# sjpark0905/DNA-LDPC-codes

Measured on AMD Instinct MI355X. Metric: decoded codewords/sec (n=18432, m=2048, 50 BP iters) at 1/2/4/8 GPUs; % HBM roofline, higher is better.
Workload: dtype f64; 1 GPU; bsc-p0.02-100k-per-gpu-bp50; code=decode_n18432_m2048_final.pchk (8,72)-regular, E=147456, input=int8 channel codes in HBM + table code*ln49 (LR = host exp), batch_per_gpu=100000, global_batch=100000, max_iter=50, algo=bp, parallelism=dp1 (contiguous codeword shards, no collective), resident_per_pass=192, group_tiles=3, nontemporal_d=False, continuous=True, resident_pool=True, syndrome_split=False

## Files before the change

dna-ldpc-codes_amd/csrc/engine.hip:

```cpp
#include <hip/hip_ext.h>
#include <hip/hip_runtime.h>

#include <algorithm>
#include <cmath>
#include <cstdio>
#include <cstdlib>
#include <cstring>
#include <thread>
#include <type_traits>
#include <utility>

#include "engine.hpp"
#include "kernels.hpp"
#include "kernels_int.hpp"
#include "encode_kernels.hpp"

namespace ldpc {

static_assert(kTile == dev::TILE && kMsaRecPlanes == dev::MSA_REC_PLANES && kMsaErShift == dev::MSA_ER_SHIFT,
              "engine_plan.hpp restates the kernels' layout constants");
constexpr int kProbes = 4;

static thread_local std::string g_err;
void set_error(const std::string& msg) { g_err = msg; }
// ... 282 lines not shown
    size_t fr = 0, tot = 0;
    if (chunk <= 0) LDPC_HIP(hipMemGetInfo(&fr, &tot));
    p = plan_engine(*g, algo, chunk, sched, fr);
    if (p.error) { set_error(p.error); return LDPC_ERR_ARG; }

    if ((rc = dg.build(*g, p.msa_c))) return rc;
    if (p.cont && (rc = lp.build(p, g->N))) return rc;
    const size_t E = (size_t)std::max<int64_t>(g->E, 1), cap = (size_t)p.cap, tiles = (size_t)p.cap_tiles, N = (size_t)g->N;
    if ((rc = dev_alloc(v2c, cap * E))) return rc;
    if (!p.res && (rc = dev_alloc(c2v_buf, p.c2v_bytes / sizeof(double)))) return rc;
    if ((rc = dev_alloc(prior, cap * N)) || (p.msa_c && (rc = dev_alloc(d_sgn, cap * N))) ||
        (rc = dev_alloc(hard, tiles * N)) || (rc = dev_alloc(active, tiles)) || (rc = dev_alloc(iters, cap)) ||
        (rc = dev_alloc(valid, cap)))
        return rc;
    if (algo < LDPC_ALGO_QMSA && (p.res || p.group_tiles < p.cap_tiles)) return probe(kProbes);
    return LDPC_OK;
}

int32_t Engine::flags() const
{
    return (p.nt_d ? LDPC_SCHED_NONTEMPORAL : 0) | (p.cont ? LDPC_SCHED_CONTINUOUS : 0) |
           (p.msa_c ? LDPC_SCHED_MSA_COMPRESSED : 0) | (p.res ? LDPC_SCHED_RESIDENT : 0) |
           (p.syn_blocks > 0 ? LDPC_SCHED_SPLIT_SYNDROME : 0) | (p.first_fp ? LDPC_SCHED_FIRST_FROM_PRIOR : 0) |
           (p.handover ? LDPC_SCHED_HANDOVER : 0) |
           (sched.flags & (LDPC_SCHED_LR_TABLE | LDPC_SCHED_DEBUG_NO_DRAIN | LDPC_SCHED_DEBUG_BAD_LANE));
}

int Engine::probe(int probes)
{
    dev_ptr<double>& pool = p.res ? v2c : c2v_buf;
    std::vector<dev_ptr<double>> cand;
    cand.push_back(std::move(pool));
    size_t best = 0;
    const int rc = time_candidates(probes, cand, &best);
    pool = std::move(cand[best]);
    return rc;
}

int Engine::time_candidates(int probes, std::vector<dev_ptr<double>>& cand, size_t* best)
{
    const size_t E = (size_t)std::max<int64_t>(g->E, 1);
    const size_t bytes = p.res ? (size_t)p.cap * E * sizeof(double) : p.c2v_bytes;
    const unsigned gt = (unsigned)(p.res ? p.cap_tiles : std::min<int64_t>(p.group_tiles, p.cap_tiles));
    hipStream_t s = stream.get();
    LDPC_HIP(hipMemsetAsync((p.res ? cand[0] : v2c).get(), 0, (size_t)gt * 64 * E * sizeof(double), s));
    LDPC_HIP(hipMemsetAsync(prior.get(), 0, (size_t)gt * 64 * g->N * sizeof(double), s));
    LDPC_HIP(hipMemsetAsync(active.get(), 0xff, (size_t)gt * sizeof(uint64_t), s));
// ... 34 lines not shown
}

int Engine::launch_check(double* scratch, int64_t t0, unsigned gt, const dev::ResStep* rstep, bool timing)
{
    using namespace dev;
    const int32_t M = g->M;
    const int64_t E = g->E;
    const bool reg72 = g->regular_dc && g->dc_max == 72;
    const dim3 grid((M + 3) / 4, gt), blk(256);
    const bool msa = algo == LDPC_ALGO_MSA;
    const int kc = timing ? K_UNCOUNTED : K_CHECK;
    int rc = LDPC_OK;
    if (rstep && !reg72) {
        const int cb = gen_bucket(g->dc_max, CheckBuckets{});
        if (!p.res || scratch != v2c.get() || t0 != 0 || !cb) { set_error("resident check: bad state"); return LDPC_ERR_ARG; }
        dispatch(cb, CheckBuckets{}, [&](auto D, auto MSA) {
            rc = launch(kc, (k_check_gr_res<MSA(), D()>), grid, blk, v2c, dg.row_ptr, M, E, *rstep);
        }, msa);
        return rc;
    }
    if (rstep) {
        if (!p.res || p.msa_c || scratch != v2c.get()) { set_error("resident check: bad state"); return LDPC_ERR_ARG; }
        if (msa) return launch(kc, (k_check_msa<72, false, true>), grid, blk, v2c, v2c, active, M, E, t0, *rstep);
        return launch(kc, (k_check_bp<72, false, true>), grid, blk, v2c, v2c, active, M, E, t0, *rstep);
    }
    if (p.msa_c) {
        const dim3 g1((unsigned)((M + 3) / 4) * gt);
        with_bools([&](auto NT) {
            rc = launch(kc, (k_check_msa_c<72, NT()>), g1, blk, v2c, msa_rec(scratch), msa_meta(scratch, p.c2v_tiles, M),
                        active, dg.row_pos, M, E, t0, gt);
        }, p.nt_d);
        return rc;
    }
    if (reg72) {
        with_bools([&](auto NT) {
            if (msa) rc = launch(kc, (k_check_msa<72, NT(), false>), grid, blk, v2c, scratch, active, M, E, t0, ResStep{});
            else rc = launch(kc, (k_check_bp<72, NT(), false>), grid, blk, v2c, scratch, active, M, E, t0, ResStep{});
        }, p.nt_d);
        return rc;
    }
    const bool bp = algo == LDPC_ALGO_BP;
    const bool in_regs = dispatch(gen_bucket(g->dc_max, CheckBuckets{}), CheckBuckets{}, [&](auto D, auto MSA) {
        rc = launch(kc, k_check_gr<MSA(), D()>, grid, blk, v2c, scratch, active, dg.row_ptr, M, E, t0);
    }, !bp);
    if (!in_regs && bp) rc = launch(kc, k_check_bp_gen, grid, blk, v2c, scratch, active, dg.row_ptr, M, E, t0);
    else if (!in_regs) rc = launch(kc, k_check_msa_gen, grid, blk, v2c, scratch, active, dg.row_ptr, M, E, t0);
// ... 9 lines not shown
int Engine::launch_var(double* scratch, int64_t t0, unsigned gt, double* pt, const dev::Refill& rf, bool timing)
{
    using namespace dev;
    const int32_t N = g->N, M = g->M;
    const int64_t E = g->E;
    const bool reg8 = g->regular_dv && g->dv_max == 8;
    const bool cnt = rf.fresh != nullptr;
    const bool pc = cnt && rf.in_code != nullptr;
    const bool inplace = scratch == v2c.get();
    const int kc = timing ? K_UNCOUNTED : K_VAR;
    int rc = LDPC_OK;
    bool ok = true;
    if (p.msa_c) {
        int cpw = std::min(var_cpw_for(rf), 4);
        if (N % (4 * cpw) != 0) cpw = 1;
        const unsigned nb = gt * (unsigned)(N / (4 * cpw));
        const double* rec = msa_rec(scratch);
        const uint16_t* meta = msa_meta(scratch, p.c2v_tiles, M);
        ok = dispatch(cpw, std::integer_sequence<int, 1, 2, 3, 4>{}, [&](auto CPW, auto CONT, auto NT, auto PC) {
            if constexpr (CONT() || !PC())
                rc = launch(kc, (k_var_msa_c<72, 8, CONT(), CPW(), NT(), PC()>), dim3(nb), dim3(256), rec, meta, v2c, prior,
                            hard, d_sgn, active, dg.col_er, pt, N, M, E, t0, (uint32_t)gt, dg.msa_pa, dg.msa_pb, rf);
        }, cnt, p.nt_d, pc);
    } else if (reg8) {
        const int want = var_cpw_for(rf);
        const int cpw = (want != 3 && N % (4 * want) == 0) ? want : 1;
        const dim3 grid((unsigned)((N + 4 * cpw - 1) / (4 * cpw)), gt);
        ok = dispatch(cpw, std::integer_sequence<int, 1, 2, 4, 8>{},
                      [&](auto CPW, auto MSA, auto NT, auto CONT, auto IP, auto PC) {
            if constexpr (!(IP() && NT()) && (CONT() || !PC()))
                rc = launch(kc, (k_var_m<MSA(), 8, NT(), CONT(), CPW(), IP(), PC()>), grid, dim3(256), scratch, v2c, prior,
                            hard, active, dg.col_edge, pt, N, E, t0, rf);
        }, algo == LDPC_ALGO_MSA, p.nt_d && !inplace, cnt, inplace, pc);
    } else {
        const dim3 grid((N + 3) / 4, gt), blk(256);
        const int vb = gen_bucket(g->dv_max, VarBuckets{});
        const bool bp = algo == LDPC_ALGO_BP;
        if (cnt) {
            if (!vb) { set_error("continuous mode needs column degrees <= 32"); return LDPC_ERR_ARG; }
            dispatch(vb, VarBuckets{}, [&](auto D, auto MSA, auto PC, auto IP) {
                rc = launch(kc, (k_var_gr_cont<MSA(), D(), PC(), IP()>), grid, blk, scratch, v2c, prior, hard, active,
                            dg.col_ptr, dg.col_edge, pt, N, E, t0, rf);
            }, algo == LDPC_ALGO_MSA, pc, inplace);
        } else {
            const bool in_regs = dispatch(vb, VarBuckets{}, [&](auto D, auto MSA) {
                rc = launch(kc, k_var_gr<MSA(), D()>, grid, blk, scratch, v2c, prior, hard, active, dg.col_ptr,
// ... 419 lines not shown
```

dna-ldpc-codes_amd/csrc/engine_plan.hpp:

```cpp
#pragma once
#include <algorithm>
#include <cmath>
#include <cstddef>
#include <cstdint>
#include <utility>

#include "../../include/ldpc_amd.h"
#include "graph.hpp"

namespace ldpc {

constexpr int32_t kDefaultGroupTiles = 3;
constexpr int32_t kDefaultMsaGroupTiles = 8;
constexpr int32_t kDefaultVarCpw = 4;
constexpr int32_t kDefaultVarCpwCoded = 2;
constexpr int32_t kDefaultPoolTiles = 3;
constexpr int32_t kDefaultResPoll = 8;
constexpr int32_t kDefaultSynBlocks = 32;
constexpr int64_t kMsaPool = 1024;
constexpr int64_t kResAutoMaxTiles = 4;

constexpr int32_t kDefaultFlags = LDPC_SCHED_NONTEMPORAL | LDPC_SCHED_CONTINUOUS | LDPC_SCHED_MSA_COMPRESSED |
                                  LDPC_SCHED_RESIDENT | LDPC_SCHED_FIRST_FROM_PRIOR | LDPC_SCHED_LR_TABLE |
                                  LDPC_SCHED_HANDOVER;
constexpr int32_t kAllFlags = kDefaultFlags | LDPC_SCHED_DEBUG_NO_DRAIN | LDPC_SCHED_DEBUG_BAD_LANE;

constexpr int32_t kResolved = 1 << 30, kResChosen = 1 << 29;

inline ldpc_schedule resolve_schedule(const ldpc_schedule* s)
{
    ldpc_schedule r{};
    if (s) r = *s;
    r.flags_set &= kAllFlags;
    r.flags = (kDefaultFlags & ~r.flags_set) | (r.flags & r.flags_set);
    r.flags &= kAllFlags;
    r.flags_set = kAllFlags | kResolved | ((r.flags_set & LDPC_SCHED_RESIDENT) ? kResChosen : 0);
    if (r.group_tiles == 0) r.group_tiles = -2;
    if (r.var_cpw < 1 || r.var_cpw > 8 || (r.var_cpw > 4 && r.var_cpw != 8)) r.var_cpw = -2;
    if (r.pool_tiles <= 0) r.pool_tiles = 0;
    if (r.poll_every <= 0) r.poll_every = kDefaultResPoll;
    if (r.syn_blocks <= 0) r.syn_blocks = kDefaultSynBlocks;
    r.syn_blocks = std::min(r.syn_blocks, 256);
    r.reserved = 0;
    return r;
}
inline bool sched_flag(const ldpc_schedule& s, int bit) { return (s.flags & bit) != 0; }

template <int... Ds>
using Buckets = std::integer_sequence<int, Ds...>;
using CheckBuckets = Buckets<8, 16, 32, 48, 64, 96>;
using VarBuckets = Buckets<4, 8, 12, 16, 24, 32>;

template <int... Ds>
inline int gen_bucket(int32_t dmax, Buckets<Ds...>)
{
    int b = 0;
    (void)((dmax <= Ds && (b = Ds, true)) || ...);
    return b;
}

constexpr double kGenPoolBytes = 226e6;
inline int32_t gen_pool_tiles(const HostGraph& g)
{
    const double per_tile = 64.0 * 8.0 * ((double)g.E + (double)g.N);
    return (int32_t)std::max(1.0, std::min(256.0, std::floor(kGenPoolBytes / std::max(per_tile, 1.0))));
}

inline int64_t engine_bytes_per_codeword(const HostGraph& g)
{
    return 2 * g.E * 8 + (int64_t)g.N * 8 + (g.N + 7) / 8 + 8;
}

constexpr int kTile = 64, kMsaRecPlanes = 4, kMsaErShift = 18;

inline size_t msa_scratch_bytes(int64_t tiles, int32_t M)
{
    return (size_t)tiles * M * kTile * (kMsaRecPlanes * sizeof(double) + sizeof(uint16_t));
}

struct EnginePlan {
    bool msa_c = false;
    bool cont = false;
    bool res = false;
    bool handover = false;
    bool nt_d = false;
    bool first_fp = false;
    bool debug_no_drain = false;
    bool debug_bad_lane = false;
    int var_cpw = 4;
    int res_poll = 8;
    int syn_blocks = 0;
    int64_t cap = 0;
    int64_t cap_tiles = 0;
    int64_t group_tiles = 0;
    int64_t c2v_tiles = 0;
    size_t c2v_bytes = 0;
    const char* error = nullptr;
};

inline EnginePlan plan_engine(const HostGraph& g, int algo, int64_t chunk, const ldpc_schedule& s, size_t free_bytes)
{
    EnginePlan p;
    const bool int_algo = algo >= LDPC_ALGO_QMSA;
    const bool reg_72_8 = g.regular_dc && g.dc_max == 72 && g.regular_dv && g.dv_max == 8;
    p.msa_c = algo == LDPC_ALGO_MSA && reg_72_8 && g.N % 16 == 0 && g.E < ((int64_t)1 << kMsaErShift) &&
              sched_flag(s, LDPC_SCHED_MSA_COMPRESSED);
    p.cont = sched_flag(s, LDPC_SCHED_CONTINUOUS) && !int_algo &&
             (reg_72_8 || (g.regular_dv && g.dv_max == 8) || gen_bucket(g.dv_max, VarBuckets{}) != 0);
    const bool gen_res = !reg_72_8 && gen_bucket(g.dc_max, CheckBuckets{}) != 0 &&
                         gen_bucket(g.dv_max, VarBuckets{}) != 0;
    p.res = sched_flag(s, LDPC_SCHED_RESIDENT) && p.cont && !p.msa_c && ((reg_72_8 && g.N % 32 == 0) || gen_res);
    const bool res_chosen = (s.flags_set & kResChosen) != 0;
    if (p.res && !res_chosen && chunk > kResAutoMaxTiles * 64) p.res = false;
    if (p.res && !res_chosen && reg_72_8 && s.pool_tiles <= 0 &&
        64.0 * 8.0 * kDefaultPoolTiles * ((double)g.E + (double)g.N) > 1.15 * kGenPoolBytes)
        p.res = false;
    p.nt_d = sched_flag(s, LDPC_SCHED_NONTEMPORAL) && !p.res;
    p.handover = sched_flag(s, LDPC_SCHED_HANDOVER) && p.res && reg_72_8 &&
                 (algo == LDPC_ALGO_BP || algo == LDPC_ALGO_MSA);
    p.debug_no_drain = sched_flag(s, LDPC_SCHED_DEBUG_NO_DRAIN);
    p.debug_bad_lane = sched_flag(s, LDPC_SCHED_DEBUG_BAD_LANE);
    p.var_cpw = s.var_cpw;
    p.res_poll = s.poll_every;
    if (chunk <= 0) {
        const int64_t ptiles = s.pool_tiles > 0 ? s.pool_tiles : reg_72_8 ? kDefaultPoolTiles : gen_pool_tiles(g);
        const int64_t want = p.res ? 64 * ptiles : (p.msa_c && p.cont) ? kMsaPool : 16384;
        chunk = std::min<int64_t>(want, (int64_t)(free_bytes / 2) / engine_bytes_per_codeword(g));
    }
    p.cap = std::max<int64_t>(64, (chunk + 63) / 64 * 64);
    p.cap_tiles = p.cap / 64;
    if (p.cap_tiles > 65535) { p.error = "chunk too large (max 4194240 codewords)"; return p; }
    int64_t group = s.group_tiles;
    if (group == -2) group = p.msa_c ? kDefaultMsaGroupTiles : kDefaultGroupTiles;
    p.group_tiles = (p.res || group <= 0 || group > p.cap_tiles) ? p.cap_tiles : group;
    if (p.cont) {
        p.syn_blocks = p.res ? 0 : s.syn_blocks;
        p.first_fp = !p.res && reg_72_8 && algo == LDPC_ALGO_BP && sched_flag(s, LDPC_SCHED_FIRST_FROM_PRIOR);
    }
    if (p.res) {
        p.c2v_tiles = p.cap_tiles;
    } else {
        p.c2v_tiles = std::max<int64_t>(p.group_tiles, p.cont ? (p.cap_tiles + 3) / 4 : 0);
// ... 8 lines not shown
```

dna-ldpc-codes_amd/csrc/kernels.hpp:

```cpp
#pragma once
#include <hip/hip_runtime.h>
#include <cstdint>

#include "kargs.hpp"

namespace ldpc {
namespace dev {

constexpr int TILE = 64;

__device__ __forceinline__ int wave_id() { return __builtin_amdgcn_readfirstlane((int)(threadIdx.x >> 6)); }
__device__ __forceinline__ int lane_id() { return (int)(threadIdx.x & 63); }

__device__ __forceinline__ unsigned xcd_block(unsigned b, unsigned nb)
{
    const unsigned q = nb / 8, r = nb % 8, x = b % 8;
    return (x < r ? x * (q + 1) : r * (q + 1) + (x - r) * q) + b / 8;
}

__device__ __forceinline__ uint64_t shfl_xor_u64(uint64_t v, int m)
{
    uint32_t lo = (uint32_t)v, hi = (uint32_t)(v >> 32);
    lo = (uint32_t)__shfl_xor((int)lo, m);
    hi = (uint32_t)__shfl_xor((int)hi, m);
// ... 325 lines not shown
    double s = 1.0;
#pragma unroll
    for (int g = NSEG - 1; g >= 0; --g) {
        double pk[SEG];
        double q = cp[g];
        asm volatile("" : "+v"(q));
#pragma unroll
        for (int i = 0; i < SEG; ++i) {
            const int k = g * SEG + i;
            if (k < DC) { pk[i] = q; q = q * x[k]; }
        }
#pragma unroll
        for (int i = SEG - 1; i >= 0; --i) {
            const int k = g * SEG + i;
            if (k < DC) {
                const double tt = pk[i] * s;
                dst[(size_t)k * TILE] = (1.0 + tt) / (1.0 - tt);
                s = s * x[k];
            }
        }
    }
}

template <int DC, bool NT, bool RES>
__device__ __forceinline__ void check_bp_block(typename Msg<RES>::in dmsg, typename Msg<RES>::out lr_t,
                                               const uint64_t* __restrict__ active, int32_t M, int64_t E,
                                               int64_t t, uint32_t rb, uint32_t nrb, const ResStep& rs)
{
    const int lane = lane_id();
    const int32_t row = (int32_t)rb * 4 + wave_id();
    const uint64_t act = RES ? rs.cs.occupied[t] : active[t];
    const auto src = dmsg + ((size_t)t * E + (size_t)row * DC) * TILE + lane;
    const auto dst = lr_t + (size_t)row * DC * TILE + lane;
    if constexpr (!RES) {
        if (!(row < M && line_occupied(act, lane))) return;
        double x[DC];
        check_bp_load<DC, NT, false>(x, src);
        check_bp_compute<DC, false>(x, dst);
    } else {
        static_assert(DC <= 2 * TILE, "row parity: two gathers per lane");
        const bool occ_l = (act >> lane) & 1ull;
        const int32_t ln0 = rs.cs.lane_n[t * TILE + lane];
        const int64_t b0 = rs.cs.lane_b[t * TILE + lane];
        const uint64_t pend = pend_lanes(rs, t);
        uint64_t par = 0;
        if (row < M && act != 0) {
            const int32_t* __restrict__ cols = rs.col_idx + (size_t)row * DC;
            const int32_t c0 = cols[lane < DC ? lane : DC - 1];
            const int32_t c1 = cols[TILE + lane < DC ? TILE + lane : DC - 1];
            double x[DC];
            check_bp_load<DC, NT, true>(x, src);
            int32_t d0 = c0, d1 = c1;
            asm volatile("" : "+v"(d0), "+v"(d1));
            const uint64_t* __restrict__ h = rs.hard + (size_t)t * rs.N;
            const uint64_t g0 = h[d0];
            const uint64_t g1 = h[d1];
            check_bp_compute<DC, true>(x, dst);
            uint64_t p = (lane < DC ? g0 : 0ull) ^ (TILE + lane < DC ? g1 : 0ull);
#pragma unroll
            for (int off = 32; off > 0; off >>= 1) p ^= shfl_xor_u64(p, off);
            par = p;
        }
        res_arrive(t, act, par, rs, occ_l ? ln0 : 0, occ_l ? b0 : 0, nrb, pend, pend_parity<DC>(rs, t, row, M, pend));
    }
}

template <int DC, bool PC = false>
__global__ __launch_bounds__(256, 2) void k_check_bp_first(const double* __restrict__ prior,
                                                           const int8_t* __restrict__ pcode,
// ... 54 lines not shown
        const int64_t b = sb[l];
        sc[l][lane] = b >= 0 ? in_code[(size_t)b * N + j0 + lane] : (int8_t)0;
    }
    __syncthreads();
    const bool fr = (frm >> lane) & 1ull;
    for (int c = w; c < TILE; c += 4) {
        const int8_t k = sc[lane][c];
        const size_t o = (size_t)t * N + j0 + c;
        pcode[o * TILE + lane] = k;
        const uint64_t m = __ballot(fr && ptab[k + kCodeBias] < 1.0);
        if (lane == 0) hard[o] = (frm == ~0ull) ? m : ((hard[o] & ~frm) | m);
    }
}

template <int DC, bool NT, bool RES>
__global__ __launch_bounds__(256, 2) void k_check_bp(typename Msg<RES>::in dmsg, typename Msg<RES>::out lr,
                                                     const uint64_t* __restrict__ active, int32_t M, int64_t E,
                                                     int64_t t0, ResStep rs)
{
    check_bp_block<DC, NT, RES>(dmsg, lr + (size_t)blockIdx.y * E * TILE, active, M, E, t0 + blockIdx.y, blockIdx.x,
                                gridDim.x, rs);
}

__global__ __launch_bounds__(256) void k_check_bp_gen(const double* __restrict__ dmsg, double* __restrict__ lr,
                                                      const uint64_t* __restrict__ active,
                                                      const int32_t* __restrict__ row_ptr, int32_t M, int64_t E,
                                                      int64_t t0)
{
    const int lane = lane_id();
    const int32_t row = blockIdx.x * 4 + wave_id();
    const int64_t t = t0 + blockIdx.y;
    if (row >= M) return;
    const uint64_t act = active[t];
    if (!((act >> lane) & 1ull)) return;
    const int32_t a = row_ptr[row], b = row_ptr[row + 1];
    const size_t tb = (size_t)t * E, tl = (size_t)blockIdx.y * E;
    double dl = 1.0;
    for (int32_t e = a; e < b; ++e) {
        lr[(tl + e) * TILE + lane] = dl;
        dl = dl * dmsg[(tb + e) * TILE + lane];
    }
    dl = 1.0;
    for (int32_t e = b - 1; e >= a; --e) {
        const size_t o = (tl + e) * TILE + lane;
        const double tt = lr[o] * dl;
        lr[o] = (1.0 + tt) / (1.0 - tt);
        dl = dl * dmsg[(tb + e) * TILE + lane];
    }
}

template <bool PC>
__device__ __forceinline__ double prior_at(const double* __restrict__ prior, const Refill& rf, size_t i)
{
    if constexpr (PC) return rf.ptab[rf.pcode[i] + kCodeBias];
    else return prior[i];
}

template <bool MSA, int DV, bool NT, bool CONT, int CPW, bool INPLACE, bool PC = false>
__device__ __forceinline__ void var_m_block(typename Msg<INPLACE>::in c2v_t, typename Msg<INPLACE>::out v2c,
                                            double* __restrict__ prior, uint64_t* __restrict__ hard,
                                            const uint64_t* __restrict__ active, const int32_t* __restrict__ col_edge,
                                            double* __restrict__ post, int32_t N, int64_t E, int64_t t, uint32_t cb,
                                            const Refill& rf)
{
    const int lane = lane_id();
    const int32_t j0 = ((int32_t)cb * 4 + wave_id()) * CPW;
    if (j0 >= N) return;
    const uint64_t act = active[t];
    const uint64_t frm = CONT ? rf.fresh[t] : 0ull;
    const uint64_t touched = act | frm;
    const uint64_t fm = (CONT && rf.fin) ? rf.fin[t] : 0ull;
    constexpr bool HO = CONT && INPLACE;
    const uint64_t lastm = (HO && rf.last) ? rf.last[t] : 0ull;
    if (touched == 0 && fm == 0) return;
    const bool live = (act >> lane) & 1ull;
    const bool fr = CONT && ((frm >> lane) & 1ull);
    const bool fl = (fm >> lane) & 1ull;
    const bool ls = HO && ((lastm >> lane) & 1ull);
// ... 22 lines not shown
            else xin[c] = rf.in[rb + j0 + c];
        }
    }
    if (live) {
#pragma unroll
        for (int c = 0; c < CPW; ++c) {
            pv[c] = prior_at<PC>(prior, rf, ((size_t)t * N + j0 + c) * TILE + lane);
#pragma unroll
            for (int s = 0; s < DV; ++s) l[c][s] = c2v_t[(size_t)eid[c][s] * TILE + lane];
        }
    }
    if constexpr (PC) {
        if (fr) {
#pragma unroll
            for (int c = 0; c < CPW; ++c) xin[c] = rf.ptab[kin[c] + kCodeBias];
        }
    }
    if (HO && lastm != 0) {
        const int64_t lb = ls ? rf.pend_b[t * TILE + lane] : 0;
        const bool lok = out_ok(lb, rf);
        uint64_t hwf[CPW];
#pragma unroll
        for (int c = 0; c < CPW; ++c) {
            bool hf = false;
            if (ls) {
                double p = pv[c];
                if (MSA) {
#pragma unroll
                    for (int s = 0; s < DV; ++s) p = p + l[c][s];
                    hf = !(p > 0);
                    if (lok && rf.post_out) rf.post_out[(size_t)lb * N + j0 + c] = p;
                } else {
#pragma unroll
                    for (int s = 0; s < DV; ++s) p = p * l[c][s];
                    if (__builtin_isnan(p)) p = 1.0;
                    hf = (p <= 1.0);
                    if (lok && rf.post_out) rf.post_out[(size_t)lb * N + j0 + c] = rf.post_ratio ? p : log(p);
                }
            }
            hwf[c] = __ballot(hf);
            if (lane == 0) rf.hard_fin[(size_t)t * N + j0 + c] = hwf[c];
        }
        if (ls && lok) store_fin_hard<CPW>(rf, hwf, lb, N, j0, lane);
        if (ls && !lok) lane_fault(rf.fault, kFaultOutput, t * TILE + lane);
    }
    const bool fok = out_ok(fb, rf);
    if (CONT && fl && fok) {
        uint64_t hw[CPW];
#pragma unroll
        for (int c = 0; c < CPW; ++c) hw[c] = hard[(size_t)t * N + j0 + c];
        store_fin_hard<CPW>(rf, hw, fb, N, j0, lane);
    }
#pragma unroll
    for (int c = 0; c < CPW; ++c) {
        const int32_t j = j0 + c;
        const size_t pj = ((size_t)t * N + j) * TILE + lane;
        if (CONT && fl && fok && rf.post_out) {
            const size_t ob = (size_t)fb * N + j;
            const double pv = fn > 0 ? post[pj] : prior_at<PC>(prior, rf, pj);
            if (MSA) rf.post_out[ob] = pv;
            else {
                const double P = __builtin_isnan(pv) ? 1.0 : pv;
                rf.post_out[ob] = rf.post_ratio ? P : log(P);
            }
        }
        bool h = false;
        double dv[DV];
#pragma unroll
        for (int s = 0; s < DV; ++s) dv[s] = 0.0;
        double np = 0.0;
        if (live) np = pv[c];
        if (fr) {
            const double x = xin[c];
            if (MSA) {
                np = x;
#pragma unroll
                for (int s = 0; s < DV; ++s) dv[s] = x;
                h = !(x > 0);
            } else {
                const double LR0 = (!PC && rf.in_is_llr) ? exp(x) : x;
                np = LR0;
                const double d0 = 1.0 - 2.0 / (1.0 + LR0);
#pragma unroll
                for (int s = 0; s < DV; ++s) dv[s] = d0;
                h = (LR0 < 1.0);
            }
        } else if (live && !ls) {
            if (MSA) {
#pragma unroll
                for (int s = 0; s < DV; ++s) {
                    double sum = pv[c];
#pragma unroll
                    for (int r = 0; r < DV; ++r)
                        if (r != s) sum = sum + l[c][r];
                    dv[s] = sum;
                }
                double L = pv[c];
#pragma unroll
                for (int s = 0; s < DV; ++s) L = L + l[c][s];
                h = !(L > 0);
                if (post) post[pj] = L;
            } else {
                double pr[DV];
                double p = pv[c];
#pragma unroll
                for (int s = 0; s < DV; ++s) { pr[s] = p; p = p * l[c][s]; }
                if (__builtin_isnan(p)) p = 1.0;
                h = (p <= 1.0);
                if (post) post[pj] = p;
                double acc = 1.0;
#pragma unroll
                for (int s = DV - 1; s >= 0; --s) {
                    double v = pr[s] * acc;
                    if (__builtin_isnan(v)) v = 1.0;
                    acc = acc * l[c][s];
                    dv[s] = 1.0 - 2.0 / (1.0 + v);
                }
            }
        }
        if (CONT && fr) {
            if constexpr (PC) rf.pcode[pj] = kin[c];
            else prior[pj] = np;
        }
        const bool skip_init = CONT && rf.prior_only && !live;
        if (!skip_init && (line_occupied(touched, lane) || fr || live)) {
#pragma unroll
            for (int s = 0; s < DV; ++s) st<NT>(v2c + (tb + eid[c][s]) * TILE + lane, dv[s]);
        }
        const uint64_t m = __ballot(h);
        if (lane == 0 && touched) {
            const size_t o = (size_t)t * N + j;
            const uint64_t old = (touched == ~0ull) ? 0ull : hard[o];
            hard[o] = (old & ~touched) | (m & touched);
        }
    }
    if (CONT && fl && !fok) lane_fault(rf.fault, kFaultOutput, t * TILE + lane);
    asm volatile("" : "+v"(bad_v));
    if (bad_v) lane_fault(rf.fault, kFaultRefill, t * TILE + lane);
}

template <bool MSA, int DV, bool NT, bool CONT, int CPW, bool INPLACE, bool PC = false>
__global__ __launch_bounds__(256) void k_var_m(typename Msg<INPLACE>::in c2v, typename Msg<INPLACE>::out v2c,
                                               double* __restrict__ prior, uint64_t* __restrict__ hard,
                                               const uint64_t* __restrict__ active,
                                               const int32_t* __restrict__ col_edge, double* __restrict__ post,
                                               int32_t N, int64_t E, int64_t t0, Refill rf)
{
    static_assert(CONT || !PC, "coded priors come with continuous refills");
    var_m_block<MSA, DV, NT, CONT, CPW, INPLACE, PC>(c2v + (size_t)blockIdx.y * E * TILE, v2c, prior, hard, active,
                                                 col_edge, post, N, E, t0 + blockIdx.y,
                                                 xcd_block(blockIdx.x, gridDim.x), rf);
}

__device__ __forceinline__ void merge_hard(uint64_t* __restrict__ hard, int64_t t, int32_t N, int32_t j, uint64_t mask,
                                           bool h, int lane)
{
    const uint64_t m = __ballot(h);
    if (lane == 0 && mask) {
        const size_t o = (size_t)t * N + j;
        const uint64_t old = (mask == ~0ull) ? 0ull : hard[o];
        hard[o] = (old & ~mask) | (m & mask);
    }
}

__global__ __launch_bounds__(256) void k_var_bp_gen(const double* __restrict__ lr, double* __restrict__ dmsg,
                                                    const double* __restrict__ prior, uint64_t* __restrict__ hard,
                                                    const uint64_t* __restrict__ active, const int32_t* __restrict__ col_ptr,
                                                    const int32_t* __restrict__ col_edge, double* __restrict__ post,
                                                    int32_t N, int64_t E, int64_t t0)
{
    const int lane = lane_id();
    const int32_t j = blockIdx.x * 4 + wave_id();
    const int64_t t = t0 + blockIdx.y;
    if (j >= N) return;
// ... 973 lines not shown
```

dna-ldpc-codes_amd/ldpc_amd.py:

```python
from __future__ import annotations

import ctypes as C
import enum
import math
import os
import threading
import time
from typing import Optional, Sequence

import numpy as np

_HERE = os.path.dirname(os.path.abspath(__file__))
LIB_PATH = os.path.join(_HERE, "lib", "libldpc_amd.so")

ABI_VERSION = 3
LDPC_OK, LDPC_ERR_ARG, LDPC_ERR_IO, LDPC_ERR_FORMAT, LDPC_ERR_DEVICE, LDPC_ERR_UNSUPPORTED = 0, -1, -2, -3, -4, -5


class Algo(enum.IntEnum):
    BP = 0
    MSA = 1
    QMSA = 2
    GALLAGER_A = 3
    GALLAGER_B1 = 4
# ... 1 lines not shown


ALGO_BP, ALGO_MSA, ALGO_QMSA = Algo.BP, Algo.MSA, Algo.QMSA
ALGO_GALLAGER_A, ALGO_GALLAGER_B1, ALGO_GALLAGER_B2 = Algo.GALLAGER_A, Algo.GALLAGER_B1, Algo.GALLAGER_B2
POST_LLR, POST_RATIO = 0, 1
IN_LLR, IN_LR = 0, 1
H2D, D2H, D2D = 0, 1, 2

_NAMES = {"bp": ALGO_BP, "msa": ALGO_MSA, "min-sum": ALGO_MSA, "qmsa": ALGO_QMSA,
          "gallager_a": ALGO_GALLAGER_A, "gallager_b1": ALGO_GALLAGER_B1, "gallager_b2": ALGO_GALLAGER_B2}
DECODER_TYPES = {0: ALGO_BP, 1: ALGO_GALLAGER_A, 2: ALGO_GALLAGER_B1, 3: ALGO_GALLAGER_B2,
                 20: ALGO_MSA, 21: ALGO_MSA, 22: ALGO_MSA}
_RESULT_TYPE = {ALGO_BP: 0, ALGO_GALLAGER_A: 1, ALGO_GALLAGER_B1: 2, ALGO_GALLAGER_B2: 3, ALGO_MSA: 20,
                ALGO_QMSA: 21}


class LdpcError(RuntimeError):
    def __init__(self, code: int, msg: str):
        super().__init__(f"ldpc_amd error {code}: {msg}")
        self.code = code


SCHED_FLAGS = {"nontemporal": 1 << 0, "continuous": 1 << 3, "msa_compressed": 1 << 4, "resident": 1 << 5,
               "split_syndrome": 1 << 6, "handover": 1 << 7, "first_from_prior": 1 << 12, "lr_table": 1 << 13,
               "debug_no_drain": 1 << 14, "debug_bad_lane": 1 << 15}
SCHED_FIELDS = ("group_tiles", "var_cpw", "pool_tiles", "poll_every", "syn_blocks")


class Schedule(C.Structure):
    _fields_ = [("flags_set", C.c_int32), ("flags", C.c_int32), ("group_tiles", C.c_int32), ("var_cpw", C.c_int32),
                ("pool_tiles", C.c_int32), ("poll_every", C.c_int32), ("syn_blocks", C.c_int32),
                ("reserved", C.c_int32)]

    @classmethod
    def make(cls, **kw) -> "Schedule":
        s = cls()
        for k, v in kw.items():
            if v is None:
                continue
            if k in SCHED_FLAGS:
                s.flags_set |= SCHED_FLAGS[k]
                if v:
                    s.flags |= SCHED_FLAGS[k]
            elif k in SCHED_FIELDS:
                setattr(s, k, int(v))
            else:
                raise TypeError(f"unknown schedule keyword {k!r} (flags: {sorted(SCHED_FLAGS)}, fields: {SCHED_FIELDS})")
# ... 440 lines not shown

class Engine:

    def __init__(self, g: Graph, device: int = 0, algo="bp", chunk: int = 0, schedule=None, **sched_kw):
        self.g, self.device, self.algo = g, device, _algo(algo)
        kw = dict(_schedule_kw(schedule))
        kw.update({k: v for k, v in sched_kw.items() if v is not None})
        sch = Schedule.make(**kw)
        err = C.c_int(0)
        self._h = lib().ldpc_engine_create_ex(g.handle, device, self.algo, chunk, C.byref(sch), C.byref(err))
        if not self._h:
            raise LdpcError(err.value, (lib().ldpc_last_error() or b"").decode())
        cap, grp, fl = C.c_int64(), C.c_int64(), C.c_int32()
        _check(lib().ldpc_engine_info(self._h, C.byref(cap), C.byref(grp), C.byref(fl)))
        self.cap, self.group_tiles, self.flags = cap.value, grp.value, fl.value
        f = fl.value
        self.nontemporal = bool(f & SCHED_FLAGS["nontemporal"])
        self.continuous = bool(f & SCHED_FLAGS["continuous"])
        self.msa_compressed = bool(f & SCHED_FLAGS["msa_compressed"])
        self.resident = bool(f & SCHED_FLAGS["resident"])
        self.syndrome_split = bool(f & SCHED_FLAGS["split_syndrome"])
        self.first_from_prior = bool(f & SCHED_FLAGS["first_from_prior"])
        self.handover = bool(f & SCHED_FLAGS["handover"])

    def decode(self, d_in, in_kind: int, B: int, max_iter: int, d_hard=None, d_post=None, post_kind=POST_LLR,
               d_iters=None, d_valid=None):
        _check(lib().ldpc_engine_decode(self._h, d_in, in_kind, B, max_iter, d_hard, d_post, post_kind, d_iters,
                                        d_valid))

    def decode_codes(self, d_codes, table: np.ndarray, table_kind: int, B: int, max_iter: int, d_hard=None,
                     d_post=None, post_kind=POST_LLR, d_iters=None, d_valid=None):
        t = np.ascontiguousarray(table, dtype=np.float64)
        if t.shape != (256,):
            raise ValueError("the code table has 256 entries (code + 128)")
        _check(lib().ldpc_engine_decode_codes(self._h, d_codes, _ptr(t), table_kind, B, max_iter, d_hard, d_post,
                                              post_kind, d_iters, d_valid))

    def set_params(self, msa_precision: int = 6, msa_step: float = 0.5, msa_offset: int = 0, tie_seed: int = 0):
        _check(lib().ldpc_engine_set_params(self._h, msa_precision, msa_step, msa_offset, tie_seed))

    def gen_bsc(self, d_out, out_kind: int, b0: int, B: int, d_cw, n_cw: int, seed: int, p: float, llr_mag: float):
        _check(lib().ldpc_engine_gen_bsc(self._h, d_out, out_kind, b0, B, d_cw, n_cw, seed, p, llr_mag))

    def gen_bsc_codes(self, d_out, b0: int, B: int, d_cw, n_cw: int, seed: int, p: float):
        _check(lib().ldpc_engine_gen_bsc_codes(self._h, d_out, b0, B, d_cw, n_cw, seed, p))

# ... 94 lines not shown
```

include/ldpc_amd.h:

```cpp
#ifndef LDPC_AMD_H
#define LDPC_AMD_H

#include <stddef.h>
#include <stdint.h>

#ifdef __cplusplus
extern "C" {
#endif

#define LDPC_AMD_ABI_VERSION 3

enum {
    LDPC_OK = 0,
    LDPC_ERR_ARG = -1,
    LDPC_ERR_IO = -2,
    LDPC_ERR_FORMAT = -3,
    LDPC_ERR_DEVICE = -4,
    LDPC_ERR_UNSUPPORTED = -5
};

enum {
    LDPC_ALGO_BP = 0,
    LDPC_ALGO_MSA = 1,
    LDPC_ALGO_QMSA = 2,
// ... 1 lines not shown
    LDPC_ALGO_GALLAGER_B1 = 4,
    LDPC_ALGO_GALLAGER_B2 = 5
};

enum {
    LDPC_POST_LLR = 0,
    LDPC_POST_RATIO = 1
};

enum {
    LDPC_IN_LLR = 0,
    LDPC_IN_LR = 1
};

typedef struct ldpc_graph ldpc_graph;

enum {
    LDPC_SCHED_NONTEMPORAL = 1 << 0,
    LDPC_SCHED_CONTINUOUS = 1 << 3,
    LDPC_SCHED_MSA_COMPRESSED = 1 << 4,
    LDPC_SCHED_RESIDENT = 1 << 5,
    LDPC_SCHED_SPLIT_SYNDROME = 1 << 6,
    LDPC_SCHED_HANDOVER = 1 << 7,
    LDPC_SCHED_FIRST_FROM_PRIOR = 1 << 12,
    LDPC_SCHED_LR_TABLE = 1 << 13,
    LDPC_SCHED_DEBUG_NO_DRAIN = 1 << 14,
    LDPC_SCHED_DEBUG_BAD_LANE = 1 << 15
};

typedef struct ldpc_schedule {
    int32_t flags_set;
    int32_t flags;
    int32_t group_tiles;
    int32_t var_cpw;
    int32_t pool_tiles;
    int32_t poll_every;
    int32_t syn_blocks;
    int32_t reserved;
} ldpc_schedule;

typedef struct ldpc_opts {
    int32_t n_devices;
    const int32_t *devices;
    int64_t chunk;
    int32_t exp_on_host;
    int32_t post_kind;
// ... 239 lines not shown
```

Measured before the change: 27750 codewords/s.

## Fuse check update of one row block into the BP variable kernel

Detects a block of M/8 check rows whose columns each appear exactly once, so every variable node has one edge there. For that block the variable kernel keeps the new variable-to-check messages in shared memory and computes the check-node BP update in the same pass with prefix and suffix products. The check kernel then only computes parity for those rows, which removes one pass over that eighth of the message array. It adds a new kernel path with 8 waves per block and a dependency on the code structure. It is on by default for resident, regular (72,8) BP when the default var_cpw is used.

```diff
diff --git a/dna-ldpc-codes_amd/csrc/engine.hip b/dna-ldpc-codes_amd/csrc/engine.hip
--- a/dna-ldpc-codes_amd/csrc/engine.hip
+++ b/dna-ldpc-codes_amd/csrc/engine.hip
@@ -328,7 +328,7 @@
     return (p.nt_d ? LDPC_SCHED_NONTEMPORAL : 0) | (p.cont ? LDPC_SCHED_CONTINUOUS : 0) |
            (p.msa_c ? LDPC_SCHED_MSA_COMPRESSED : 0) | (p.res ? LDPC_SCHED_RESIDENT : 0) |
            (p.syn_blocks > 0 ? LDPC_SCHED_SPLIT_SYNDROME : 0) | (p.first_fp ? LDPC_SCHED_FIRST_FROM_PRIOR : 0) |
-           (p.handover ? LDPC_SCHED_HANDOVER : 0) |
+           (p.handover ? LDPC_SCHED_HANDOVER : 0) | (p.fuse_block >= 0 ? LDPC_SCHED_FUSE_ROW_BLOCK : 0) |
            (sched.flags & (LDPC_SCHED_LR_TABLE | LDPC_SCHED_DEBUG_NO_DRAIN | LDPC_SCHED_DEBUG_BAD_LANE));
 }
 
@@ -409,6 +409,12 @@
     if (rstep) {
         if (!p.res || p.msa_c || scratch != v2c.get()) { set_error("resident check: bad state"); return LDPC_ERR_ARG; }
         if (msa) return launch(kc, (k_check_msa<72, false, true>), grid, blk, v2c, v2c, active, M, E, t0, *rstep);
+        if (p.fuse_block >= 0) {
+            if (t0 != 0) { set_error("resident check: bad state"); return LDPC_ERR_ARG; }
+            const int32_t Q = M / 8;
+            return launch(kc, (k_check_bp_skip<72>), grid, blk, v2c, v2c, M, E, p.fuse_block * Q, (p.fuse_block + 1) * Q,
+                          *rstep);
+        }
         return launch(kc, (k_check_bp<72, false, true>), grid, blk, v2c, v2c, active, M, E, t0, *rstep);
     }
     if (p.msa_c) {
@@ -464,6 +470,13 @@
                 rc = launch(kc, (k_var_msa_c<72, 8, CONT(), CPW(), NT(), PC()>), dim3(nb), dim3(256), rec, meta, v2c, prior,
                             hard, d_sgn, active, dg.col_er, pt, N, M, E, t0, (uint32_t)gt, dg.msa_pa, dg.msa_pb, rf);
         }, cnt, p.nt_d, pc);
+    } else if (reg8 && p.fuse_block >= 0 && cnt && inplace) {
+        if (t0 != 0 || timing) { set_error("fused row block: bad state"); return LDPC_ERR_ARG; }
+        const dim3 grid((unsigned)(M / 8), gt);
+        with_bools([&](auto PC) {
+            rc = launch(kc, (k_var_bp_fused<kFuseWaves, kFuseCpw, PC()>), grid, dim3(64 * kFuseWaves), v2c, prior, hard,
+                        active, dg.col_edge, dg.col_idx, pt, N, E, p.fuse_block * (M / 8), rf);
+        }, pc);
     } else if (reg8) {
         const int want = var_cpw_for(rf);
         const int cpw = (want != 3 && N % (4 * want) == 0) ? want : 1;
diff --git a/dna-ldpc-codes_amd/csrc/engine_plan.hpp b/dna-ldpc-codes_amd/csrc/engine_plan.hpp
--- a/dna-ldpc-codes_amd/csrc/engine_plan.hpp
+++ b/dna-ldpc-codes_amd/csrc/engine_plan.hpp
@@ -4,6 +4,7 @@
 #include <cstddef>
 #include <cstdint>
 #include <utility>
+#include <vector>
 
 #include "../../include/ldpc_amd.h"
 #include "graph.hpp"
@@ -25,16 +26,18 @@
                                   LDPC_SCHED_HANDOVER;
 constexpr int32_t kAllFlags = kDefaultFlags | LDPC_SCHED_DEBUG_NO_DRAIN | LDPC_SCHED_DEBUG_BAD_LANE;
 
-constexpr int32_t kResolved = 1 << 30, kResChosen = 1 << 29;
+constexpr int32_t kResolved = 1 << 30, kResChosen = 1 << 29, kNoFuse = 1 << 28;
 
 inline ldpc_schedule resolve_schedule(const ldpc_schedule* s)
 {
     ldpc_schedule r{};
     if (s) r = *s;
+    const bool no_fuse = (r.flags_set & LDPC_SCHED_FUSE_ROW_BLOCK) && !(r.flags & LDPC_SCHED_FUSE_ROW_BLOCK);
     r.flags_set &= kAllFlags;
     r.flags = (kDefaultFlags & ~r.flags_set) | (r.flags & r.flags_set);
     r.flags &= kAllFlags;
-    r.flags_set = kAllFlags | kResolved | ((r.flags_set & LDPC_SCHED_RESIDENT) ? kResChosen : 0);
+    r.flags_set = kAllFlags | kResolved | ((r.flags_set & LDPC_SCHED_RESIDENT) ? kResChosen : 0) |
+                  (no_fuse ? kNoFuse : 0);
     if (r.group_tiles == 0) r.group_tiles = -2;
     if (r.var_cpw < 1 || r.var_cpw > 8 || (r.var_cpw > 4 && r.var_cpw != 8)) r.var_cpw = -2;
     if (r.pool_tiles <= 0) r.pool_tiles = 0;
@@ -78,11 +81,32 @@
     return (size_t)tiles * M * kTile * (kMsaRecPlanes * sizeof(double) + sizeof(uint16_t));
 }
 
+inline int fuse_row_block_of(const HostGraph& g)
+{
+    const int dv = g.dv_max;
+    if (dv <= 0 || g.M % dv != 0 || !g.regular_dc) return -1;
+    const int32_t Q = g.M / dv;
+    if ((int64_t)Q * g.dc_max != g.N) return -1;
+    std::vector<uint8_t> seen((size_t)g.N);
+    for (int a = 0; a < dv; a++) {
+        std::fill(seen.begin(), seen.end(), (uint8_t)0);
+        bool once = true;
+        for (int64_t e = (int64_t)a * Q * g.dc_max; once && e < (int64_t)(a + 1) * Q * g.dc_max; e++) {
+            uint8_t& c = seen[(size_t)g.col_idx[(size_t)e]];
+            once = c == 0;
+            c = 1;
+        }
+        if (once) return a;
+    }
+    return -1;
+}
+
 struct EnginePlan {
     bool msa_c = false;
     bool cont = false;
     bool res = false;
     bool handover = false;
+    int fuse_block = -1;
     bool nt_d = false;
     bool first_fp = false;
     bool debug_no_drain = false;
@@ -118,6 +142,8 @@
     p.nt_d = sched_flag(s, LDPC_SCHED_NONTEMPORAL) && !p.res;
     p.handover = sched_flag(s, LDPC_SCHED_HANDOVER) && p.res && reg_72_8 &&
                  (algo == LDPC_ALGO_BP || algo == LDPC_ALGO_MSA);
+    if (!(s.flags_set & kNoFuse) && p.res && reg_72_8 && algo == LDPC_ALGO_BP && s.var_cpw == -2)
+        p.fuse_block = fuse_row_block_of(g);
     p.debug_no_drain = sched_flag(s, LDPC_SCHED_DEBUG_NO_DRAIN);
     p.debug_bad_lane = sched_flag(s, LDPC_SCHED_DEBUG_BAD_LANE);
     p.var_cpw = s.var_cpw;
diff --git a/dna-ldpc-codes_amd/csrc/kernels.hpp b/dna-ldpc-codes_amd/csrc/kernels.hpp
--- a/dna-ldpc-codes_amd/csrc/kernels.hpp
+++ b/dna-ldpc-codes_amd/csrc/kernels.hpp
@@ -371,11 +371,13 @@
     }
 }
 
-template <int DC, bool NT, bool RES>
+template <int DC, bool NT, bool RES, bool SKIP = false>
 __device__ __forceinline__ void check_bp_block(typename Msg<RES>::in dmsg, typename Msg<RES>::out lr_t,
                                                const uint64_t* __restrict__ active, int32_t M, int64_t E,
-                                               int64_t t, uint32_t rb, uint32_t nrb, const ResStep& rs)
-{
+                                               int64_t t, uint32_t rb, uint32_t nrb, const ResStep& rs,
+                                               int32_t skip_lo = 0, int32_t skip_hi = 0)
+{
+    static_assert(RES || !SKIP, "rows are skipped in the resident pool only");
     const int lane = lane_id();
     const int32_t row = (int32_t)rb * 4 + wave_id();
     const uint64_t act = RES ? rs.cs.occupied[t] : active[t];
@@ -393,7 +395,9 @@
         const int64_t b0 = rs.cs.lane_b[t * TILE + lane];
         const uint64_t pend = pend_lanes(rs, t);
         uint64_t par = 0;
-        if (row < M && act != 0) {
+        if (SKIP && row >= skip_lo && row < skip_hi) {
+            if (act != 0) par = row_parity<DC>(rs.hard + (size_t)t * rs.N, rs.col_idx + (size_t)row * DC);
+        } else if (row < M && act != 0) {
             const int32_t* __restrict__ cols = rs.col_idx + (size_t)row * DC;
             const int32_t c0 = cols[lane < DC ? lane : DC - 1];
             const int32_t c1 = cols[TILE + lane < DC ? TILE + lane : DC - 1];
@@ -494,6 +498,14 @@
                                 gridDim.x, rs);
 }
 
+template <int DC>
+__global__ __launch_bounds__(256, 2) void k_check_bp_skip(const double* dmsg, double* lr, int32_t M, int64_t E,
+                                                          int32_t skip_lo, int32_t skip_hi, ResStep rs)
+{
+    check_bp_block<DC, false, true, true>(dmsg, lr + (size_t)blockIdx.y * E * TILE, nullptr, M, E, blockIdx.y,
+                                          blockIdx.x, gridDim.x, rs, skip_lo, skip_hi);
+}
+
 __global__ __launch_bounds__(256) void k_check_bp_gen(const double* __restrict__ dmsg, double* __restrict__ lr,
                                                       const uint64_t* __restrict__ active,
                                                       const int32_t* __restrict__ row_ptr, int32_t M, int64_t E,
@@ -526,6 +538,111 @@
 {
     if constexpr (PC) return rf.ptab[rf.pcode[i] + kCodeBias];
     else return prior[i];
+}
+
+template <bool MSA, int DV>
+__device__ __forceinline__ bool var_column_final(bool ls, double pvc, const double (&l)[DV], bool lok,
+                                                 const Refill& rf, int64_t lb, int32_t N, int32_t j)
+{
+    bool hf = false;
+    if (ls) {
+        double p = pvc;
+        if (MSA) {
+#pragma unroll
+            for (int s = 0; s < DV; ++s) p = p + l[s];
+            hf = !(p > 0);
+            if (lok && rf.post_out) rf.post_out[(size_t)lb * N + j] = p;
+        } else {
+#pragma unroll
+            for (int s = 0; s < DV; ++s) p = p * l[s];
+            if (__builtin_isnan(p)) p = 1.0;
+            hf = (p <= 1.0);
+            if (lok && rf.post_out) rf.post_out[(size_t)lb * N + j] = rf.post_ratio ? p : log(p);
+        }
+    }
+    return hf;
+}
+
+template <bool MSA, bool PC>
+__device__ __forceinline__ void var_column_fin_post(const Refill& rf, const double* __restrict__ prior,
+                                                    const double* post, size_t pj, size_t ob, int32_t fn)
+{
+    const double pv = fn > 0 ? post[pj] : prior_at<PC>(prior, rf, pj);
+    if (MSA) rf.post_out[ob] = pv;
+    else {
+        const double P = __builtin_isnan(pv) ? 1.0 : pv;
+        rf.post_out[ob] = rf.post_ratio ? P : log(P);
+    }
+}
+
+template <bool MSA, int DV, bool PC>
+__device__ __forceinline__ void var_column(bool live, bool fr, bool ls, double pvc, double x, const double (&l)[DV],
+                                           const Refill& rf, double* post, size_t pj, double (&dv)[DV], double& np,
+                                           bool& h)
+{
+    h = false;
+#pragma unroll
+    for (int s = 0; s < DV; ++s) dv[s] = 0.0;
+    np = 0.0;
+    if (live) np = pvc;
+    if (fr) {
+        if (MSA) {
+            np = x;
+#pragma unroll
+            for (int s = 0; s < DV; ++s) dv[s] = x;
+            h = !(x > 0);
+        } else {
+            const double LR0 = (!PC && rf.in_is_llr) ? exp(x) : x;
+            np = LR0;
+            const double d0 = 1.0 - 2.0 / (1.0 + LR0);
+#pragma unroll
+            for (int s = 0; s < DV; ++s) dv[s] = d0;
+            h = (LR0 < 1.0);
+        }
+    } else if (live && !ls) {
+        if (MSA) {
+#pragma unroll
+            for (int s = 0; s < DV; ++s) {
+                double sum = pvc;
+#pragma unroll
+                for (int r = 0; r < DV; ++r)
+                    if (r != s) sum = sum + l[r];
+                dv[s] = sum;
+            }
+            double L = pvc;
+#pragma unroll
+            for (int s = 0; s < DV; ++s) L = L + l[s];
+            h = !(L > 0);
+            if (post) post[pj] = L;
+        } else {
+            double pr[DV];
+            double p = pvc;
+#pragma unroll
+            for (int s = 0; s < DV; ++s) { pr[s] = p; p = p * l[s]; }
+            if (__builtin_isnan(p)) p = 1.0;
+            h = (p <= 1.0);
+            if (post) post[pj] = p;
+            double acc = 1.0;
+#pragma unroll
+            for (int s = DV - 1; s >= 0; --s) {
+                double v = pr[s] * acc;
+                if (__builtin_isnan(v)) v = 1.0;
+                acc = acc * l[s];
+                dv[s] = 1.0 - 2.0 / (1.0 + v);
+            }
+        }
+    }
+}
+
+__device__ __forceinline__ void merge_touched(uint64_t* __restrict__ hard, int64_t t, int32_t N, int32_t j,
+                                              uint64_t touched, bool h, int lane)
+{
+    const uint64_t m = __ballot(h);
+    if (lane == 0 && touched) {
+        const size_t o = (size_t)t * N + j;
+        const uint64_t old = (touched == ~0ull) ? 0ull : hard[o];
+        hard[o] = (old & ~touched) | (m & touched);
+    }
 }
 
 template <bool MSA, int DV, bool NT, bool CONT, int CPW, bool INPLACE, bool PC = false>
@@ -594,22 +711,7 @@
         uint64_t hwf[CPW];
 #pragma unroll
         for (int c = 0; c < CPW; ++c) {
-            bool hf = false;
-            if (ls) {
-                double p = pv[c];
-                if (MSA) {
-#pragma unroll
-                    for (int s = 0; s < DV; ++s) p = p + l[c][s];
-                    hf = !(p > 0);
-                    if (lok && rf.post_out) rf.post_out[(size_t)lb * N + j0 + c] = p;
-                } else {
-#pragma unroll
-                    for (int s = 0; s < DV; ++s) p = p * l[c][s];
-                    if (__builtin_isnan(p)) p = 1.0;
-                    hf = (p <= 1.0);
-                    if (lok && rf.post_out) rf.post_out[(size_t)lb * N + j0 + c] = rf.post_ratio ? p : log(p);
-                }
-            }
+            const bool hf = var_column_final<MSA, DV>(ls, pv[c], l[c], lok, rf, lb, N, j0 + c);
             hwf[c] = __ballot(hf);
             if (lane == 0) rf.hard_fin[(size_t)t * N + j0 + c] = hwf[c];
         }
@@ -627,69 +729,11 @@
     for (int c = 0; c < CPW; ++c) {
         const int32_t j = j0 + c;
         const size_t pj = ((size_t)t * N + j) * TILE + lane;
-        if (CONT && fl && fok && rf.post_out) {
-            const size_t ob = (size_t)fb * N + j;
-            const double pv = fn > 0 ? post[pj] : prior_at<PC>(prior, rf, pj);
-            if (MSA) rf.post_out[ob] = pv;
-            else {
-                const double P = __builtin_isnan(pv) ? 1.0 : pv;
-                rf.post_out[ob] = rf.post_ratio ? P : log(P);
-            }
-        }
-        bool h = false;
-        double dv[DV];
-#pragma unroll
-        for (int s = 0; s < DV; ++s) dv[s] = 0.0;
-        double np = 0.0;
-        if (live) np = pv[c];
-        if (fr) {
-            const double x = xin[c];
-            if (MSA) {
-                np = x;
-#pragma unroll
-                for (int s = 0; s < DV; ++s) dv[s] = x;
-                h = !(x > 0);
-            } else {
-                const double LR0 = (!PC && rf.in_is_llr) ? exp(x) : x;
-                np = LR0;
-                const double d0 = 1.0 - 2.0 / (1.0 + LR0);
-#pragma unroll
-                for (int s = 0; s < DV; ++s) dv[s] = d0;
-                h = (LR0 < 1.0);
-            }
-        } else if (live && !ls) {
-            if (MSA) {
-#pragma unroll
-                for (int s = 0; s < DV; ++s) {
-                    double sum = pv[c];
-#pragma unroll
-                    for (int r = 0; r < DV; ++r)
-                        if (r != s) sum = sum + l[c][r];
-                    dv[s] = sum;
-                }
-                double L = pv[c];
-#pragma unroll
-                for (int s = 0; s < DV; ++s) L = L + l[c][s];
-                h = !(L > 0);
-                if (post) post[pj] = L;
-            } else {
-                double pr[DV];
-                double p = pv[c];
-#pragma unroll
-                for (int s = 0; s < DV; ++s) { pr[s] = p; p = p * l[c][s]; }
-                if (__builtin_isnan(p)) p = 1.0;
-                h = (p <= 1.0);
-                if (post) post[pj] = p;
-                double acc = 1.0;
-#pragma unroll
-                for (int s = DV - 1; s >= 0; --s) {
-                    double v = pr[s] * acc;
-                    if (__builtin_isnan(v)) v = 1.0;
-                    acc = acc * l[c][s];
-                    dv[s] = 1.0 - 2.0 / (1.0 + v);
-                }
-            }
-        }
+        if (CONT && fl && fok && rf.post_out)
+            var_column_fin_post<MSA, PC>(rf, prior, post, pj, (size_t)fb * N + j, fn);
+        bool h;
+        double dv[DV], np;
+        var_column<MSA, DV, PC>(live, fr, ls, pv[c], xin[c], l[c], rf, post, pj, dv, np, h);
         if (CONT && fr) {
             if constexpr (PC) rf.pcode[pj] = kin[c];
             else prior[pj] = np;
@@ -699,12 +743,7 @@
 #pragma unroll
             for (int s = 0; s < DV; ++s) st<NT>(v2c + (tb + eid[c][s]) * TILE + lane, dv[s]);
         }
-        const uint64_t m = __ballot(h);
-        if (lane == 0 && touched) {
-            const size_t o = (size_t)t * N + j;
-            const uint64_t old = (touched == ~0ull) ? 0ull : hard[o];
-            hard[o] = (old & ~touched) | (m & touched);
-        }
+        merge_touched(hard, t, N, j, touched, h, lane);
     }
     if (CONT && fl && !fok) lane_fault(rf.fault, kFaultOutput, t * TILE + lane);
     asm volatile("" : "+v"(bad_v));
@@ -722,6 +761,154 @@
     var_m_block<MSA, DV, NT, CONT, CPW, INPLACE, PC>(c2v + (size_t)blockIdx.y * E * TILE, v2c, prior, hard, active,
                                                  col_edge, post, N, E, t0 + blockIdx.y,
                                                  xcd_block(blockIdx.x, gridDim.x), rf);
+}
+
+constexpr int kFuseWaves = 8, kFuseCpw = 3;
+template <int W, int CPW, bool PC>
+__global__ __launch_bounds__(64 * W) void k_var_bp_fused(double* msg, double* __restrict__ prior,
+                                                         uint64_t* __restrict__ hard,
+                                                         const uint64_t* __restrict__ active,
+                                                         const int32_t* __restrict__ col_edge,
+                                                         const int32_t* __restrict__ col_idx, double* post, int32_t N,
+                                                         int64_t E, int32_t row0, Refill rf)
+{
+    constexpr int DC = 72, DV = 8, KW = DC / W;
+    static_assert(DC % W == 0 && KW % CPW == 0, "the row's columns split evenly over the waves and their rounds");
+    __shared__ double sd[DC][TILE];
+    const int lane = lane_id(), w = wave_id();
+    const int64_t t = blockIdx.y;
+    const int32_t row = row0 + (int32_t)xcd_block(blockIdx.x, gridDim.x);
+    const uint64_t act = active[t];
+    const uint64_t frm = rf.fresh[t];
+    const uint64_t touched = act | frm;
+    const uint64_t fm = rf.fin ? rf.fin[t] : 0ull;
+    const uint64_t lastm = rf.last ? rf.last[t] : 0ull;
+    if (touched == 0 && fm == 0) return;
+    const bool live = (act >> lane) & 1ull;
+    const bool fr = (frm >> lane) & 1ull;
+    const bool fl = (fm >> lane) & 1ull;
+    const bool ls = (lastm >> lane) & 1ull;
+    int64_t fb = 0;
+    int32_t fn = 0;
+    if (fl) {
+        fb = rf.fin_b[t * TILE + lane];
+        fn = rf.fin_n[t * TILE + lane];
+    }
+    double* m_t = msg + (size_t)t * E * TILE;
+    const int k0 = w * KW;
+    const int32_t e0 = row * DC + k0;
+    bool bad_in = false;
+    int bad_v = 0;
+    size_t rb = 0;
+    if (fr) {
+        rb = (size_t)refill_row(rf.lane_b[t * TILE + lane], rf, bad_in) * N;
+        bad_v = bad_in ? 1 : 0;
+    }
+    const int64_t lb = ls ? rf.pend_b[t * TILE + lane] : 0;
+    const bool lok = out_ok(lb, rf), fok = out_ok(fb, rf);
+    const bool keep = line_occupied(touched, lane) || fr || live;
+#pragma unroll
+    for (int r = 0; r < KW; r += CPW) {
+        int32_t j[CPW], eid[CPW][DV];
+#pragma unroll
+        for (int c = 0; c < CPW; ++c) j[c] = col_idx[e0 + r + c];
+#pragma unroll
+        for (int c = 0; c < CPW; ++c)
+#pragma unroll
+            for (int s = 0; s < DV; ++s) eid[c][s] = col_edge[(size_t)j[c] * DV + s];
+        double l[CPW][DV], pv[CPW], xin[CPW];
+        int8_t kin[CPW];
+        if (fr) {
+#pragma unroll
+            for (int c = 0; c < CPW; ++c) {
+                if constexpr (PC) kin[c] = rf.in_code[rb + j[c]];
+                else xin[c] = rf.in[rb + j[c]];
+            }
+        }
+        if (live) {
+#pragma unroll
+            for (int c = 0; c < CPW; ++c) {
+                pv[c] = prior_at<PC>(prior, rf, ((size_t)t * N + j[c]) * TILE + lane);
+#pragma unroll
+                for (int s = 0; s < DV; ++s) l[c][s] = m_t[(size_t)eid[c][s] * TILE + lane];
+            }
+        }
+        if constexpr (PC) {
+            if (fr) {
+#pragma unroll
+                for (int c = 0; c < CPW; ++c) xin[c] = rf.ptab[kin[c] + kCodeBias];
+            }
+        }
+        if (lastm != 0) {
+#pragma unroll
+            for (int c = 0; c < CPW; ++c) {
+                const uint64_t hwf = __ballot(var_column_final<false, DV>(ls, pv[c], l[c], lok, rf, lb, N, j[c]));
+                if (lane == 0) rf.hard_fin[(size_t)t * N + j[c]] = hwf;
+                if (ls && lok) store_fin_hard<1>(rf, &hwf, lb, N, j[c], lane);
+            }
+        }
+        if (fl && fok) {
+#pragma unroll
+            for (int c = 0; c < CPW; ++c) {
+                const uint64_t hw = hard[(size_t)t * N + j[c]];
+                store_fin_hard<1>(rf, &hw, fb, N, j[c], lane);
+            }
+        }
+#pragma unroll
+        for (int c = 0; c < CPW; ++c) {
+            const size_t pj = ((size_t)t * N + j[c]) * TILE + lane;
+            if (fl && fok && rf.post_out) var_column_fin_post<false, PC>(rf, prior, post, pj, (size_t)fb * N + j[c], fn);
+            bool h;
+            double dv[DV], np;
+            var_column<false, DV, PC>(live, fr, ls, pv[c], xin[c], l[c], rf, post, pj, dv, np, h);
+            if (fr) {
+                if constexpr (PC) rf.pcode[pj] = kin[c];
+                else prior[pj] = np;
+            }
+            const int32_t ea = e0 + r + c;
+            if (keep) {
+#pragma unroll
+                for (int s = 0; s < DV; ++s) {
+                    if (eid[c][s] == ea) sd[k0 + r + c][lane] = dv[s];
+                    else m_t[(size_t)eid[c][s] * TILE + lane] = dv[s];
+                }
+            }
+            merge_touched(hard, t, N, j[c], touched, h, lane);
+        }
+    }
+    if (lastm != 0 && ls && !lok) lane_fault(rf.fault, kFaultOutput, t * TILE + lane);
+    if (fl && !fok) lane_fault(rf.fault, kFaultOutput, t * TILE + lane);
+    asm volatile("" : "+v"(bad_v));
+    if (bad_v) lane_fault(rf.fault, kFaultRefill, t * TILE + lane);
+    __syncthreads();
+    if (touched == 0) return;
+    double p = 1.0;
+    for (int g = 0; g < w; ++g) {
+        double y[KW];
+#pragma unroll
+        for (int i = 0; i < KW; ++i) y[i] = sd[g * KW + i][lane];
+#pragma unroll
+        for (int i = 0; i < KW; ++i) p = p * y[i];
+    }
+    double x[KW], pk[KW];
+#pragma unroll
+    for (int i = 0; i < KW; ++i) x[i] = sd[k0 + i][lane];
+#pragma unroll
+    for (int i = 0; i < KW; ++i) { pk[i] = p; p = p * x[i]; }
+    double sfx = 1.0;
+    for (int g = W - 1; g > w; --g) {
+        double y[KW];
+#pragma unroll
+        for (int i = 0; i < KW; ++i) y[i] = sd[g * KW + i][lane];
+#pragma unroll
+        for (int i = KW - 1; i >= 0; --i) sfx = sfx * y[i];
+    }
+#pragma unroll
+    for (int i = KW - 1; i >= 0; --i) {
+        const double tt = pk[i] * sfx;
+        if (keep) m_t[(size_t)(e0 + i) * TILE + lane] = (1.0 + tt) / (1.0 - tt);
+        sfx = sfx * x[i];
+    }
 }
 
 __device__ __forceinline__ void merge_hard(uint64_t* __restrict__ hard, int64_t t, int32_t N, int32_t j, uint64_t mask,
diff --git a/dna-ldpc-codes_amd/ldpc_amd.py b/dna-ldpc-codes_amd/ldpc_amd.py
--- a/dna-ldpc-codes_amd/ldpc_amd.py
+++ b/dna-ldpc-codes_amd/ldpc_amd.py
@@ -47,7 +47,7 @@
 
 
 SCHED_FLAGS = {"nontemporal": 1 << 0, "continuous": 1 << 3, "msa_compressed": 1 << 4, "resident": 1 << 5,
-               "split_syndrome": 1 << 6, "handover": 1 << 7, "first_from_prior": 1 << 12, "lr_table": 1 << 13,
+               "split_syndrome": 1 << 6, "handover": 1 << 7, "fuse_row_block": 1 << 8, "first_from_prior": 1 << 12, "lr_table": 1 << 13,
                "debug_no_drain": 1 << 14, "debug_bad_lane": 1 << 15}
 SCHED_FIELDS = ("group_tiles", "var_cpw", "pool_tiles", "poll_every", "syn_blocks")
 
@@ -534,6 +534,7 @@
         self.syndrome_split = bool(f & SCHED_FLAGS["split_syndrome"])
         self.first_from_prior = bool(f & SCHED_FLAGS["first_from_prior"])
         self.handover = bool(f & SCHED_FLAGS["handover"])
+        self.fused_row_block = bool(f & SCHED_FLAGS["fuse_row_block"])
 
     def decode(self, d_in, in_kind: int, B: int, max_iter: int, d_hard=None, d_post=None, post_kind=POST_LLR,
                d_iters=None, d_valid=None):
diff --git a/include/ldpc_amd.h b/include/ldpc_amd.h
--- a/include/ldpc_amd.h
+++ b/include/ldpc_amd.h
@@ -47,6 +47,7 @@
     LDPC_SCHED_RESIDENT = 1 << 5,
     LDPC_SCHED_SPLIT_SYNDROME = 1 << 6,
     LDPC_SCHED_HANDOVER = 1 << 7,
+    LDPC_SCHED_FUSE_ROW_BLOCK = 1 << 8,
     LDPC_SCHED_FIRST_FROM_PRIOR = 1 << 12,
     LDPC_SCHED_LR_TABLE = 1 << 13,
     LDPC_SCHED_DEBUG_NO_DRAIN = 1 << 14,
```

Result: faster. 28320 codewords/s (median of 6 runs) (+2.1%).
